# YonghaoHe/LFD-A-Light-and-Fast-Detector

Hardware: AMD Instinct MI355X
Metric: images/sec WIDERFACE-S 1920x1080 bs=8 end-to-end inference, LFD.precision='fp32_storage' (raw logits within 1e-4 of fp32: inside north_star's 1e-3; the 'fp16' mode, sigma 2.5e-3, under fp16_mode) (higher is better)
Workload: dtype f16

## Files before the change

### include/lfd_hip.h

```cpp
#ifndef LFD_HIP_H_
#define LFD_HIP_H_

#include <stddef.h>
#include <stdint.h>

#ifdef __cplusplus
extern "C" {
#endif

#define LFD_HIP_ABI_VERSION 3
#define LFD_MAX_LEVELS 8

typedef void* lfd_stream_t;

#if defined(LFD_BUILDING)
#define LFD_API __attribute__((visibility("default")))
#else
#define LFD_API
#endif

enum lfd_status {
  LFD_OK = 0,
  LFD_ERR_INVALID_ARGUMENT = -1,
  LFD_ERR_WORKSPACE_TOO_SMALL = -2,
// ... 201 lines not shown
                                    const float* b2, const void* zeros, lfd_stream_t stream);

LFD_API int lfd_upsample_nearest_add_nhwc_f16(void* dst, const void* src, int32_t n, int32_t H, int32_t W, int32_t h,
                                              int32_t w, int32_t c, lfd_stream_t stream);
LFD_API int lfd_relu_inplace_f16(void* x, int64_t count, lfd_stream_t stream);
LFD_API int lfd_maxpool3x3s2_nhwc_f16(const void* in, void* out, int32_t n, int32_t h, int32_t w, int32_t c,
                                      lfd_stream_t stream);
LFD_API int lfd_pack_level_outputs_f32(const float* src, float* dst, int32_t n, int32_t hw, int32_t src_channels, int32_t c0,
                                       int32_t count, int32_t total_points, int32_t point_offset, float scale, int32_t op,
                                       lfd_stream_t stream);

LFD_API int lfd_conv2d_nhwc_f16_acc32(const lfd_conv_desc_t* desc, const void* in, float* out_f32, const void* w_packed,
                                      const float* bias, const void* zeros, lfd_stream_t stream);

typedef struct lfd_p32_conv_desc {
  int32_t n, h, w, cin, cout, ks, stride, relu;
  int32_t in_format;
  int32_t out_pixel_stride;
  int64_t out_image_stride;
} lfd_p32_conv_desc_t;
LFD_API size_t lfd_p32_conv_packed_weight_halfs(int32_t cin, int32_t cout, int32_t ks);
LFD_API int lfd_p32_conv2d_nhwc_f32(const lfd_p32_conv_desc_t* desc, const void* in, float* out, const void* w_packed,
                                    const float* bias, const float* residual, const float* scale, lfd_stream_t stream);
LFD_API int lfd_p32_conv2d_tail_nhwc_f32(const lfd_p32_conv_desc_t* desc, const void* in, float* out, const void* w_packed,
                                         const float* bias, const void* tail_w_packed, const float* tail_bias, int32_t tail_relu,
                                         lfd_stream_t stream);
LFD_API size_t lfd_p32_groupnorm_workspace_bytes(int32_t n, int32_t groups);
LFD_API int lfd_p32_groupnorm_relu_f32(float* x, int32_t n, int64_t hw, int32_t c, int32_t groups, const float* gamma,
                                       const float* beta, float eps, int32_t relu, void* workspace, size_t workspace_bytes,
                                       lfd_stream_t stream);

#define LFD_PL_GN_REPLICAS 8
typedef struct lfd_pl_conv_desc {
  int32_t n, h, w, cin, cout, ks, stride, relu;
  int32_t tail_cout, tail_relu;
  int32_t out_mode;
  int32_t f_c0, f_c1;
  float gn_in_eps;
  int64_t in_plane_halfs, out_plane_halfs, res_plane_halfs, ds_plane_halfs;
  int64_t f_image_stride0, f_image_stride1;
} lfd_pl_conv_desc_t;
LFD_API int lfd_pl_stem_pair(const void* in, int32_t in_format, int32_t n, int32_t h, int32_t w, int32_t channels,
                             const void* w1_packed, const float* b1, const void* w2_packed, const float* b2, void* out,
                             int64_t out_plane_halfs, lfd_stream_t stream);
LFD_API int lfd_pl_stem2x(const void* in, int32_t in_format, int32_t n, int32_t h, int32_t w, const void* w1_packed,
                          const void* w2_packed, const float* b2, const void* w3_packed, const float* b3,
                          const void* w4_packed, const float* b4, void* out, int64_t out_plane_halfs, const void* zeros,
                          lfd_stream_t stream);
LFD_API int lfd_pl_conv2d(const lfd_pl_conv_desc_t* desc, const void* in, void* out, const void* w_packed, const float* bias,
                          const void* residual, const void* tail_w_packed, const float* tail_bias, const void* ds_w_packed,
                          const float* ds_bias, void* ds_out, void* gn_sums, float* f_out0, float* f_out1, const float* scale1,
                          const void* gn_in_sums, const float* gn_in_gamma, const float* gn_in_beta, const void* zeros,
                          lfd_stream_t stream);
typedef struct lfd_pl_level {
  const void* in;
  void* out;
  const void* w_packed;
  const float* bias;
  const void* tail_w_packed;
  const float* tail_bias;
  void* gn_sums;
  const void* gn_in_sums;
  const float* gn_in_gamma;
  const float* gn_in_beta;
  float* f_out0;
  float* f_out1;
  const float* scale1;
  int32_t h, w;
  int64_t in_plane_halfs, out_plane_halfs;
} lfd_pl_level_t;
LFD_API int lfd_pl_conv2d_levels(const lfd_pl_conv_desc_t* desc, const lfd_pl_level_t* levels, int32_t num_levels,
                                 const void* zeros, lfd_stream_t stream);
LFD_API int lfd_pl_groupnorm_relu(void* x, int64_t plane_halfs, int32_t n, int64_t hw, int32_t c, const void* gn_sums,
                                  const float* gamma, const float* beta, float eps, int32_t relu, lfd_stream_t stream);

typedef struct lfd_pl_head_desc {
  int32_t mode, n, cin, relu0;
  int32_t f_c0, f_c1;
  float gn_in_eps;
  int32_t pad_;
  int64_t f_image_stride0, f_image_stride1;
} lfd_pl_head_desc_t;
typedef struct lfd_pl_head_level {
  const void* in;
  void* out;
  const void* w0;
  const float* b0;
  const void* w1;
  const float* b1;
  void* gn_sums;
  const void* gn_in_sums;
  const float* gn_in_gamma;
  const float* gn_in_beta;
  float* f_out0;
  float* f_out1;
  const float* scale1;
  int64_t in_plane_halfs;
  int32_t pixels, pad_;
} lfd_pl_head_level_t;
LFD_API int lfd_pl_head_levels(const lfd_pl_head_desc_t* desc, const lfd_pl_head_level_t* levels, int32_t num_levels,
                               const void* zeros, lfd_stream_t stream);

LFD_API int lfd_stem_conv_f16(const void* in, int32_t in_format, int32_t n, int32_t h, int32_t w,
                              int32_t channels, const void* w1_packed, const float* b1,
                              const void* w2_packed, const float* b2, void* out, lfd_stream_t stream);

// ... 232 lines not shown
```

### lfd-a-light-and-fast-detector_amd/lfd_amd/_lib.py

```python
import ctypes as C
import os

_HERE = os.path.dirname(os.path.abspath(__file__))
LIB_PATH = os.environ.get('LFD_HIP_LIB') or os.path.join(_HERE, 'liblfd_hip.so')
MAX_LEVELS = 8
F32, F16 = 0, 1

_lib = None


class DetectDesc(C.Structure):
    _fields_ = [('num_levels', C.c_int32),
                ('level_h', C.c_int32 * MAX_LEVELS), ('level_w', C.c_int32 * MAX_LEVELS),
                ('level_stride', C.c_int32 * MAX_LEVELS),
                ('level_range_lo', C.c_float * MAX_LEVELS), ('level_range_hi', C.c_float * MAX_LEVELS),
                ('num_classes', C.c_int32), ('num_cls_channels', C.c_int32),
                ('score_mode', C.c_int32), ('decode_mode', C.c_int32),
                ('class_agnostic', C.c_int32), ('max_candidates', C.c_int32),
                ('score_thr', C.c_float), ('iou_thr', C.c_float)]


class DetectExt(C.Structure):
    _fields_ = [('pre_nms_limit', C.c_int32), ('post_nms_limit', C.c_int32)]

# ... 174 lines not shown
    'lfd_gn_train_stats_f16': (C.c_int, [_P, _I32, _I64, _I32, _I32, _F, _P, _SZ, _P, _P]),
    'lfd_gn_train_apply_f16': (C.c_int, [_P, _I32, _I64, _I32, _I32, _P, _P, _P, _I32, _P, _P]),
    'lfd_gn_train_stats_apply_f16': (C.c_int, [_P, _I32, _I64, _I32, _I32, _F, _P, _P, _I32, _P, _SZ, _P, _P, _P]),
    'lfd_gn_train_stats_apply_seg_f16': (C.c_int, [_P, _I32, _I32, _P, _I32, _I32, _F, _P, _P, _I32, _P, _SZ, _P, _P, _P]),
    'lfd_gn_train_bwd_seg_f16': (C.c_int, [_P, _P, _P, _I32, _I32, _P, _I32, _I32, _P, _P, _F, _I32, _P, _SZ, _P, _P, _P, _P]),
    'lfd_bn_train_apply_into_f16': (C.c_int, [_P, _I32, _I64, _I32, _P, _P, _P, _I32, _P, _I64, _I64, _P]),
    'lfd_bn_train_bwd_from_f16': (C.c_int, [_P, _I64, _I64, _P, _I32, _I32, _I64, _I32, _P, _P, _P, _F, _I32, _P, _SZ, _P, _P, _P, _P]),
    'lfd_head_out_split_concat_f16': (C.c_int, [_P, _I32, _I32, _I64, _I64, C.POINTER(HeadOutSeg), _I32, _P]),
    'lfd_head_out_grad_concat_f16': (C.c_int, [_P, _I32, _I32, _I64, _I64, C.POINTER(HeadOutSeg), _I32, _F, _P, _P, _SZ, _P]),
    'lfd_conv2d_bn_partials_nhwc_f16': (C.c_int, [C.POINTER(ConvDesc), _P, _P, _P, _P, _P, _P, _SZ, C.POINTER(C.c_int32), _P]),
    'lfd_bn_train_finish_into_levels_f16': (C.c_int, [C.POINTER(BnFwdLevel), _I32, _I32, _I32, _P, _I64, _P]),
    'lfd_bn_train_bwd_from_levels_f16': (C.c_int, [_P, _I64, C.POINTER(BnBwdLevel), _I32, _I32, _I32, _F, _I32, _P, _SZ, _P]),
    'lfd_head_out_split_levels_f16': (C.c_int, [_P, _I32, _I64, C.POINTER(HeadOutLevel), _I32, _P]),
    'lfd_head_out_grad_levels_f16': (C.c_int, [_P, _I32, _I64, C.POINTER(HeadOutLevel), _I32, _F, _P, _P, _SZ, _P]),
    'lfd_gn_train_bwd_f16': (C.c_int, [_P, _P, _P, _I32, _I64, _I32, _I32, _P, _P, _F, _I32, _P, _SZ, _P, _P, _P, _P]),
    'lfd_zero_insert2_nhwc_f16': (C.c_int, [_P, _I32, _I32, _I32, _I32, _I32, _I32, _P, _P]),
    'lfd_conv3x3s2_dgrad_nhwc_f16': (C.c_int, [_I32, _I32, _I32, _P, _P, _P, _P, _P]),
    'lfd_conv_wgrad_nhwc_f16': (C.c_int, [_P, _P, _I32, _I32, _I32, _I32, _I32, _I32, _I32, _F, _I32, _P, _SZ, _P, _P]),
    'lfd_conv_wgrad_partial_rows': (_I32, [_I32, _I32, _I32, _I32, _I32, _I32, _I32]),
    'lfd_conv_wgrad_partials_nhwc_f16': (C.c_int, [_P, _P, _I32, _I32, _I32, _I32, _I32, _I32, _I32, _P, _SZ, _P]),
    'lfd_conv1x1_wgrad_partials_of_bn_relu_f16': (C.c_int, [_P, _P, _P, _P, _P, _I32, _I32, _I32, _I32, _I32, _P, _SZ, _P]),
    'lfd_wgrad_final_batched_f32': (C.c_int, [_P, _I32, _I32, _P]),
    'lfd_rows_sum_batched_f32': (C.c_int, [_P, _I32, _P]),
    'lfd_stem_conv0_train_fwd': (C.c_int, [_P, _I32, _I32, _I32, _I32, _P, _P, _P]),
    'lfd_head_out_split_f16': (C.c_int, [_P, _I32, _I32, _I64, _I64, C.POINTER(HeadOutSeg), _I32, _P]),
    'lfd_head_out_grad_f16': (C.c_int, [_P, _I32, _I32, _I64, _I64, C.POINTER(HeadOutSeg), _I32, _F, _P, _P, _SZ, _P]),
    'lfd_stem_conv0_train_fwd_bn_stats': (C.c_int, [_P, _I32, _I32, _I32, _I32, _P, _P, _F, _F, _P, _P, _P, _SZ, _P, _P]),
    'lfd_stem_conv0_wgrad': (C.c_int, [_P, _P, _I32, _I32, _I32, _I32, _F, _I32, _P, _SZ, _P, _P]),
    'lfd_stem_conv0_bn_bwd_wgrad': (C.c_int, [_P, _P, _P, _I32, _I32, _I32, _I32, _P, _P, _P, _F, _I32, _P, _SZ, _P, _P, _P, _P]),
    'lfd_stem_conv0_bn_bwd_wgrad_rows': (C.c_int, [_P, _P, _P, _I32, _I32, _I32, _I32, _P, _P, _P, _F, _I32, _I32, _P, _SZ, _P, _P, _P, _P]),
    'lfd_bn_train_bwd_rows_f16': (C.c_int, [_P, _P, _I64, _I32, _P, _P, _P, _F, _I32, _I32, _P, _SZ, _P, _P, _P, _P]),
    'lfd_conv1x1_dgrad_bn_bwd_sums_nhwc_f16': (C.c_int, [C.POINTER(ConvDesc), _P, _P, _P, _P, _P, _P, _P, _P, _P, _P, _SZ, C.POINTER(C.c_int32), _P]),
    'lfd_stem_conv_f16': (C.c_int, [_P, _I32, _I32, _I32, _I32, _I32, _P, _P, _P, _P, _P, _P]),
    'lfd_stem_faster_fused_f16': (C.c_int, [_P, _I32, _I32, _I32, _I32, _I32, _P, _P, _P, _P, _P, _P, _P, _P, _P, _P]),
    'lfd_head_partial_floats': (_SZ, [C.POINTER(HeadDesc)]),
    'lfd_head_forward_f16': (C.c_int, [C.POINTER(HeadDesc), _I32, C.POINTER(HeadLevelPtrs), _P, _P, _P, _P, _P, _P, _P]),
    'lfd_head_forward_decode_f16': (C.c_int, [C.POINTER(HeadDesc), C.POINTER(HeadLevelPtrs), _P, _P, _P, _P, _P,
                                              C.POINTER(DetectDesc), _P, _P, _SZ, _P]),
    'lfd_groupnorm_finalize': (C.c_int, [C.POINTER(HeadDesc), _P, C.POINTER(C.c_void_p), C.POINTER(C.c_void_p), _F, _P, _P]),
    'lfd_groupnorm_finalize_fold': (C.c_int, [C.POINTER(HeadDesc), _P, C.POINTER(C.c_void_p), C.POINTER(C.c_void_p), _F, _P,
                                              C.POINTER(HeadLevelPtrs), _I32, _P]),
    'lfd_conv_packed_weight_halfs': (_SZ, [_I32, _I32, _I32]),
    'lfd_conv2d_nhwc_f16': (C.c_int, [C.POINTER(ConvDesc), _P, _P, _P, _P, _P, _P, _P, _P, _P]),
    'lfd_fasterblock_fused_f16': (C.c_int, [_I32, _I32, _I32, _P, _P, _P, _P, _P, _P, _P, _P]),
    'lfd_fasterblock128_fused_f16': (C.c_int, [_I32, _I32, _I32, _P, _P, _P, _P, _P, _P, _P]),
    'lfd_downblock_fused_f16': (C.c_int, [_I32, _I32, _I32, _P, _P, _P, _P, _P, _P, _P, _P, _P, _P]),
    'lfd_conv2d_nhwc_f16_acc32': (C.c_int, [C.POINTER(ConvDesc), _P, _P, _P, _P, _P, _P]),
    'lfd_p32_conv_packed_weight_halfs': (_SZ, [_I32, _I32, _I32]),
    'lfd_p32_conv2d_nhwc_f32': (C.c_int, [C.POINTER(P32ConvDesc), _P, _P, _P, _P, _P, _P, _P]),
    'lfd_p32_conv2d_tail_nhwc_f32': (C.c_int, [C.POINTER(P32ConvDesc), _P, _P, _P, _P, _P, _P, _I32, _P]),
    'lfd_pl_stem_pair': (C.c_int, [_P, _I32, _I32, _I32, _I32, _I32, _P, _P, _P, _P, _P, _I64, _P]),
    'lfd_pl_stem2x': (C.c_int, [_P, _I32, _I32, _I32, _I32, _P, _P, _P, _P, _P, _P, _P, _P, _I64, _P, _P]),
    'lfd_pl_conv2d': (C.c_int, [C.POINTER(PlConvDesc), _P, _P, _P, _P, _P, _P, _P, _P, _P, _P, _P, _P, _P, _P, _P, _P, _P, _P, _P]),
    'lfd_pl_conv2d_levels': (C.c_int, [C.POINTER(PlConvDesc), C.POINTER(PlLevel), _I32, _P, _P]),
    'lfd_pl_head_levels': (C.c_int, [C.POINTER(PlHeadDesc), C.POINTER(PlHeadLevel), _I32, _P, _P]),
    'lfd_pl_groupnorm_relu': (C.c_int, [_P, _I64, _I32, _I64, _I32, _P, _P, _P, _F, _I32, _P]),
    'lfd_p32_groupnorm_workspace_bytes': (_SZ, [_I32, _I32]),
    'lfd_p32_groupnorm_relu_f32': (C.c_int, [_P, _I32, _I64, _I32, _I32, _P, _P, _F, _I32, _P, _SZ, _P]),
    'lfd_conv2d_downsample_nhwc_f16': (C.c_int, [C.POINTER(ConvDesc), _P, _P, _P, _P, _P, _P, _P, _P, _P]),
}


TUNE_KEYS = {'HEAD2': 0, 'H2_CHUNK': 1, 'H2_AGPR': 2, 'H2_A1': 3, 'STEM2X': 4, 'X2_ALN': 5, 'X2_STAGGER': 6, 'BLOCK_ROWS': 7,
             'ROWS_WGS': 8, 'CONV128_SPLITK': 9, 'CONV0_VALU': 10, 'PL_C3': 11, 'PL_HEAD_OUT_REGS': 12, 'PL_HEAD_ROLES': 13, 'PL_STEM': 14}


def tune(name, value=None):
    key = TUNE_KEYS[name]
    prev = lib().lfd_tuning_get(key)
    if value is not None:
        check(lib().lfd_tuning_set(key, int(value)), 'lfd_tuning_set')
    return prev


def declared_symbols():
    return sorted(_SIGNATURES)


def lib():
    global _lib
    if _lib is None:
        if not os.path.exists(LIB_PATH):
            raise RuntimeError(
                'liblfd_hip.so not found at %s -- build it with `python __graft_entry__.py` '
                '(hipcc --offload-arch=gfx950); lfd_amd has no CPU/PyTorch fallback.' % LIB_PATH)
        import torch
        l = C.CDLL(LIB_PATH)
        for name, (res, args) in _SIGNATURES.items():
            fn = getattr(l, name)
            fn.restype, fn.argtypes = res, args
        if l.lfd_hip_abi_version() != ABI_VERSION:
            raise RuntimeError('liblfd_hip.so ABI version mismatch: %s reports %d, this package binds version %d '
                               '(struct layouts differ -- rebuild with `python __graft_entry__.py`)'
                               % (LIB_PATH, l.lfd_hip_abi_version(), ABI_VERSION))
        for name, key in TUNE_KEYS.items():
            v = os.environ.get('LFD_' + name)
            if v is not None and v.strip().lstrip('-').isdigit():
                l.lfd_tuning_set(key, int(v))
        _lib = l
    return _lib


def check(status, what):
    if status != 0:
        raise RuntimeError('%s failed: %s (status %d)' % (what, lib().lfd_hip_status_string(status).decode(), status))

# ... 15 lines not shown
```

### lfd-a-light-and-fast-detector_amd/lfd_amd/engine_p2.py

```python
import ctypes as C
import os

import torch
import torch.nn as nn

from . import _lib, engine, ops
from ._lib import check, lib, ptr, stream_ptr

_UNION = engine._UNION
_LO = 2048.0


class Unsupported(Exception):
    pass


def _split(w):
    w = w.detach().float()
    hi = w.half()
    lo = ((w - hi.float()) * _LO).half()
    return hi, lo


def pack_planes_weight(w):
# ... 1 lines not shown
    cout = w.shape[0]
    ns = -(-cout // 32)
    if ns * 32 != cout:
        w = torch.cat([w, w.new_zeros((ns * 32 - cout,) + tuple(w.shape[1:]))], 0)
    hi, lo = _split(w)
    return torch.stack([ops.pack_conv_weight(hi), ops.pack_conv_weight(lo)], 0).contiguous()


def pack_planes_stem_weight(w):
    hi, lo = _split(w)
    return torch.stack([engine.pack_stem_weight(hi), engine.pack_stem_weight(lo)], 0).contiguous()


def pack_planes_stem2x_weight(w, b):
    if tuple(w.shape) != (64, 3, 3, 3) or b.numel() != 64:
        raise Unsupported('fused stem: conv0 must be [64, 3, 3, 3]')
    c = 64
    wr = w.detach().float().permute(0, 2, 3, 1).reshape(c // 32, 32, 3, 9)
    out = torch.zeros(c // 32, 2, 2, 32, 8, dtype=torch.float32, device=w.device)
    out[:, 0, 0, :, 1:] = wr[:, :, 0, :7]
    out[:, 0, 1, :, 1:] = wr[:, :, 2, :7]
    out[:, 1, 0, :, 1:] = wr[:, :, 1, :7]
    for r in range(3):
        out[:, 1, 1, :, 2 * r:2 * r + 2] = wr[:, :, r, 7:9]
    out[:, 1, 1, :, 6] = b.detach().float().reshape(c // 32, 32).to(w.device)
    hi, lo = _split(out.reshape(c // 32, 2, 64, 8))
    return torch.stack([hi, lo], 0).contiguous()


def pack_planes_stem2x_tail_weight(w):
    if tuple(w.shape) != (64, 64, 1, 1):
        raise Unsupported('fused stem: first 1x1 must be [64, 64, 1, 1]')
    w2 = w.detach().float().reshape(64, 64)
    idx = torch.empty(4, 2, 8, dtype=torch.long)
    for q in range(4):
        s_, u = q // 2, q % 2
        for hh in range(2):
            for j in range(8):
                idx[q, hh, j] = 32 * s_ + 16 * u + (4 * hh + j if j < 4 else 8 + 4 * hh + j - 4)
    g = w2[:, idx.reshape(-1).to(w2.device)].reshape(2, 32, 4, 2, 8)
    out = g.permute(0, 2, 3, 1, 4).reshape(2, 4, 64, 8)
    hi, lo = _split(out)
    return torch.stack([hi, lo], 0).contiguous()


def _flat_head_enabled():
    return os.environ.get('LFD_P2_FLATHEAD', '1') != '0'


def _stem2x_enabled():
    return os.environ.get('LFD_P2_STEM2X', '1') != '0'


def _pad_bias(b, mult=32):
    n = -(-b.numel() // mult) * mult
    out = b.new_zeros(n, dtype=torch.float32)
    out[:b.numel()] = b.float()
    return out


def to_planes(x):
    hi = x.half()
    return torch.stack([hi, ((x - hi.float()) * _LO).half()], 0).contiguous()


def from_planes(p):
    return p[0].float() + p[1].float() / _LO


_DISPATCH = {
    (64, 3, 1, 2): {'res'}, (64, 3, 2, 2): {'tail', 'ds'}, (64, 3, 2, 4): {'ds'}, (64, 1, 1, 4): {'tail', 'gn', 'out32'},
    (128, 3, 1, 4): {'res'}, (128, 3, 2, 4): {'ds'}, (128, 1, 1, 4): {'tail', 'gn', 'out32'}, (128, 1, 1, 1): {'out32'},
    (128, 1, 1, 2): {'out32'}, (32, 3, 2, 1): {'tail', 'ds'}, (32, 3, 2, 2): {'tail', 'ds'},
}


def _check_dispatch(cin, cout, ks, stride, tail, ds, res, gn, out32):
    opts = _DISPATCH.get((cin, ks, stride, -(-cout // 32)))
    used = {k for k, v in (('tail', tail), ('ds', ds), ('res', res), ('gn', gn), ('out32', out32)) if v}
    if opts is None or not (used - {'gn'} <= opts and (not gn or 'gn' in opts)) or len(used - {'gn'}) > 1:
        raise Unsupported('no plane kernel for conv %d -> %d k%d s%d %s' % (cin, cout, ks, stride, sorted(used)))
    if gn and (res or ds or out32):
        raise Unsupported('GroupNorm sums ride on a plain or chained 1x1')


def _fork_enabled():
    import os
    return os.environ.get('LFD_P2_FORK', '0') != '0'


def _levels_enabled():
    return os.environ.get('LFD_P2_LEVELS', '1') != '0'


class _Op(object):
    __slots__ = ('kind', 'src', 'dst', 'res', 'ds_dst', 'cin', 'cout', 'ks', 'stride', 'relu', 'w', 'b', 'tail', 'ds',
                 'out_mode', 'gn', 'gnin', 'level', 'f_c0', 'f_c1', 'scale', 'w1', 'b1', 'w2', 'b2', 'channels')

    def __init__(self, kind):
        self.kind = kind
        for k in self.__slots__[1:]:
            setattr(self, k, None)


class PlanesPlan(object):

    def __init__(self, model, device):
        self.device = device
        self.param_sig = engine._param_signature(model._backbone, model._neck, model._head)
        self._shape_cache = {}
        self.ops = []
        self.buf_channels = {}
        self.buf_scale = {}
        self._nbuf = 0
        self.num_gn = 0
        self.head_start = None
        self.level_ops = []
        self.tap_ready = []
        with torch.no_grad():
            self._build(model)

    def _new_buf(self, channels, scale):
        b = self._nbuf
        self._nbuf += 1
        self.buf_channels[b], self.buf_scale[b] = channels, scale
        return b

    def _conv(self, src, w, b, ks, stride, relu, res=None, tail=None, ds=None, gn=False, out32=None, gnin=None):
        dev = self.device
        cout, cin = w.shape[0], w.shape[1]
        if cin not in (32, 64, 128) or (out32 is None and cout % 32):
            raise Unsupported('conv %d -> %d' % (cin, cout))
        _check_dispatch(cin, cout, ks, stride, tail is not None, ds is not None, res is not None, gn, out32 is not None)
        o = _Op('conv')
        if gnin is not None:
            norm = gnin[1]
            if not (isinstance(norm, nn.GroupNorm) and norm.num_channels == 128 and norm.num_groups == 16 and cin == 128 and ks == 1
                    and stride == 1 and tail is None and res is None and ds is None):
                raise Unsupported('head norm must be GroupNorm(16, 128) in front of a 1x1 conv')
            o.gnin = (gnin[0], norm.weight.detach().float().contiguous().to(dev), norm.bias.detach().float().contiguous().to(dev),
                      float(norm.eps))
        o.src, o.res, o.ks, o.stride, o.relu, o.cin, o.cout = src, res, ks, stride, int(relu), cin, cout
        o.w = pack_planes_weight(w).to(dev)
        o.b = _pad_bias(b, 128).to(dev)
        sc = self.buf_scale[src] * stride
        if tail is not None:
            if tuple(tail[0].shape) != (cout, cout, 1, 1):
                raise Unsupported('chained 1x1 must be square')
            o.tail = (pack_planes_weight(tail[0]).to(dev), _pad_bias(tail[1], 128).to(dev), int(tail[2]))
        if ds is not None:
            if tuple(ds[0].shape) != (cout, cin, 1, 1) or ks != 3 or stride != 2:
                raise Unsupported('identity branch must be the 1x1 stride-2 twin of a 3x3 stride-2 conv')
            o.ds = (pack_planes_weight(ds[0]).to(dev), _pad_bias(ds[1], 128).to(dev))
            o.ds_dst = self._new_buf(cout, sc)
        if out32 is not None:
            o.out_mode = 2
            o.level, o.f_c0, o.f_c1, o.scale = out32
        else:
            o.out_mode = 1 if gn else 0
            o.dst = self._new_buf(cout, sc)
            if gn:
                if cout != 128:
                    raise Unsupported('GroupNorm sums: 128 channels in groups of 8')
                o.gn = self.num_gn
                self.num_gn += 1
        self.ops.append(o)
        return o

    def _build(self, model):
        bb, neck, head = model._backbone, model._neck, model._head
        if type(neck).__name__ != 'SimpleNeck' or type(head).__name__ != 'LFDHead':
# ... 6 lines not shown
                        'Conv2d', 'BatchNorm2d', 'GroupNorm', 'ReLU', 'Scale', 'Identity', 'Sequential', 'ModuleList'):
                    raise Unsupported('module %s (activation must be ReLU)' % type(mod).__name__)
        has_norm = bb._norm_cfg is not None
        step = 3 if has_norm else 2
        spec = list(bb.stem_spec())
        folded = [engine.fold_conv_norm(bb._stem[i * step], bb._stem[i * step + 1] if has_norm else None) for i in range(len(spec))]
        if len(spec) not in (2, 4) or [(k, s) for k, s, _, _ in spec] != [(3, 2), (1, 1)] * (len(spec) // 2):
            raise Unsupported('stem mode')
        c = folded[0][0].shape[0]
        if c not in (32, 64) or tuple(folded[1][0].shape[:2]) != (c, c):
            raise Unsupported('stem channels')
        o = _Op('stem')
        o.channels = c
        o.w1, o.b1 = pack_planes_stem_weight(folded[0][0]).to(self.device), _pad_bias(folded[0][1]).to(self.device)
        o.w2, o.b2 = pack_planes_weight(folded[1][0]).to(self.device), _pad_bias(folded[1][1]).to(self.device)
        o.dst = self._new_buf(c, 2)
        self.ops.append(o)
        cur = o.dst
        self.stem2x = None
        if len(spec) == 4:
            if tuple(folded[3][0].shape[:2]) != (c, c):
                raise Unsupported('stem channels')
            pair2 = self._conv(cur, folded[2][0], folded[2][1], 3, 2, True, tail=(folded[3][0], folded[3][1], True))
            cur = pair2.dst
            if c == 64:
                f = _Op('stem2x')
                f.w1 = pack_planes_stem2x_weight(folded[0][0], folded[0][1]).to(self.device)
                f.w2, f.b2 = pack_planes_stem2x_tail_weight(folded[1][0]).to(self.device), o.b2
                f.dst = cur
                f.tail = pair2
                self.stem2x = f
        taps = [tuple(t) for t in bb._out_indices]
        self.taps = []
        for i, nblk in enumerate(bb._body_architecture):
            for j in range(nblk):
                blk = getattr(bb, 'stage%d' % i)[j]
                ident, y = cur, cur
                for ci in range(1, blk.num_convs + 1):
                    conv = getattr(blk, '_conv%d' % ci)
                    w, b = engine.fold_conv_norm(conv, getattr(blk, '_norm%d' % ci, None))
                    ks, st = conv.kernel_size[0], conv.stride[0]
                    last = ci == blk.num_convs
                    ds = None
                    if ci == 1 and blk._downsample is not None:
                        dconv = blk._downsample[0]
                        if dconv.kernel_size[0] != 1 or dconv.stride[0] != 2 or (ks, st) != (3, 2) or last:
                            raise Unsupported('downsample branch')
                        ds = engine.fold_conv_norm(dconv, blk._downsample[1] if len(blk._downsample) > 1 else None)
                    elif ci > 1 and st != 1:
                        raise Unsupported('stride inside a block')
                    if ci == 1 and blk._downsample is None and st != 1:
                        raise Unsupported('strided block without a downsample branch')
                    op = self._conv(y, w, b, ks, st, True, res=ident if last else None, ds=ds)
                    y = op.dst
                    if ds is not None:
                        ident = op.ds_dst
                cur = y
                if (i, j) in taps:
                    self.taps.append(cur)
                    self.tap_ready.append(len(self.ops) - 1)
        if head._norm_cfg is None or head._conv_kernel_size != 1:
            raise Unsupported('head towers must be 1x1 conv + GroupNorm')
        nl = head._num_conv_layers
        union = head._regression_loss_type in _UNION
        self.cls_channels = head.num_cls_channels
        self.num_levels = head._num_heads
        ccls = self.cls_channels

        def tower(seq, t, first_tail_of=None):
            pend = None
            for l in range(nl):
                conv, norm = seq[l * 3], seq[l * 3 + 1]
                if not isinstance(norm, nn.GroupNorm):
                    raise Unsupported('head norm must be GroupNorm')
                if not isinstance(seq[l * 3 + 2], nn.ReLU):
                    raise Unsupported('head activation must be ReLU')
                bias = conv.bias.detach().float() if conv.bias is not None else torch.zeros(conv.out_channels, device=conv.weight.device)
                w = conv.weight.detach().float()
                if l == 0 and first_tail_of is not None:
                    nw, nb, src = first_tail_of
                    op = self._conv(src, nw, nb, 1, 1, True, tail=(w, bias, False), gn=True)
                else:
                    op = self._conv(t, w, bias, 1, 1, False, gn=True, gnin=pend)
                pend = (op.gn, norm)
                t = op.dst
            return t, pend

        self.head_start = len(self.ops)
        for i, f in enumerate(self.taps):
            first_op = len(self.ops)
            nseq = getattr(neck, 'neck%d' % i)
            nw, nb = engine.fold_conv_norm(nseq[0], nseq[1] if neck._norm_cfg is not None else None)
            if nw.shape[0] != 128 or nw.shape[2] != 1:
                raise Unsupported('neck must be 1x1 -> 128')
            cls_path = getattr(head, 'head%d_classification_path' % i)
            reg_path = getattr(head, 'head%d_regression_path' % i)
            scale = head._scales[i]._scale.detach().float().reshape(1).to(self.device) if union else None
            if head._merge_path_flag:
                if nl < 1:
                    raise Unsupported('merge path without tower convs')
                tt, pend = tower(getattr(head, 'head%d_merge_path' % i), None, first_tail_of=(nw, nb, f))
                cconv, rconv = cls_path[0], reg_path[0]
                if cconv.kernel_size[0] != 1 or rconv.kernel_size[0] != 1 or ccls + 4 > 64:
                    raise Unsupported('output convs')
                w = torch.cat([cconv.weight.detach().float(), rconv.weight.detach().float()], 0)
                b = torch.cat([cconv.bias.detach().float(), rconv.bias.detach().float()], 0)
# ... 157 lines not shown
                    d.mode, d.n, d.cin, d.relu0 = mode, st.n, o.cin, o.relu
                    if mode == 0:
                        lv.w1, lv.b1 = o.tail[0].data_ptr(), o.tail[1].data_ptr()
                    if mode != 2:
                        lv.out, lv.gn_sums = st.bufs[o.dst].data_ptr(), st.gn_sums[o.gn].data_ptr()
                    if gi is not None:
                        lv.gn_in_sums, lv.gn_in_gamma, lv.gn_in_beta = st.gn_sums[gi[0]].data_ptr(), gi[1].data_ptr(), gi[2].data_ptr()
                        d.gn_in_eps = gi[3]
                    if mode == 2:
                        d.f_c0, d.f_c1 = o.f_c0, o.f_c1
                        d.f_image_stride0, d.f_image_stride1 = st.P * o.f_c0, st.P * 4
                        lv.f_out0 = (st.cls.data_ptr() + st.p_off[o.level] * o.f_c0 * 4) if o.f_c0 else None
                        lv.f_out1 = (st.reg.data_ptr() + st.p_off[o.level] * 4 * 4) if o.f_c1 else None
                        lv.scale1 = o.scale.data_ptr() if o.scale is not None else None
                calls.append((mode, d, arr, len(grp)))
            st.flat_calls = calls
        for mode, d, arr, n in st.flat_calls:
            if mode == 'G':
                check(l.lfd_pl_conv2d_levels(C.byref(d), arr, n, zeros, sp), 'lfd_pl_conv2d_levels')
            else:
                check(l.lfd_pl_head_levels(C.byref(d), arr, n, zeros, sp), 'lfd_pl_head_levels')

    def _launch_levels(self, st):
        modes = self._flat_head_modes() if _flat_head_enabled() else None
        if modes is not None:
            return self._launch_levels_flat(st, modes)
        l, sp = lib(), stream_ptr()
        zeros = ptr(ops.zero_line(self.device))
        if st.level_calls is None:
            calls = []
            for grp in self.level_groups:
                arr = (_lib.PlLevel * len(grp))()
                d0 = None
                for j, i in enumerate(grp):
                    o = self.ops[i]
                    d, src, dst, _, _, f0, f1 = self._desc(o, st)
                    d0 = d0 or d
                    lv, gi = arr[j], o.gnin
                    lv.in_, lv.out, lv.w_packed, lv.bias = src.data_ptr(), dst.data_ptr() if dst is not None else None, o.w.data_ptr(), o.b.data_ptr()
                    if o.tail is not None:
                        lv.tail_w_packed, lv.tail_bias = o.tail[0].data_ptr(), o.tail[1].data_ptr()
                    if o.gn is not None:
                        lv.gn_sums = st.gn_sums[o.gn].data_ptr()
                    if gi is not None:
                        lv.gn_in_sums, lv.gn_in_gamma, lv.gn_in_beta = st.gn_sums[gi[0]].data_ptr(), gi[1].data_ptr(), gi[2].data_ptr()
                    lv.f_out0, lv.f_out1 = f0, f1
                    lv.scale1 = o.scale.data_ptr() if o.scale is not None else None
                    lv.h, lv.w, lv.in_plane_halfs, lv.out_plane_halfs = src.shape[2], src.shape[3], d.in_plane_halfs, d.out_plane_halfs
                calls.append((d0, arr, len(grp)))
            st.level_calls = calls
        for d, arr, n in st.level_calls:
            check(l.lfd_pl_conv2d_levels(C.byref(d), arr, n, zeros, sp), 'lfd_pl_conv2d_levels')

    def _launch(self, x, fmt, st, indices):
        l, sp = lib(), stream_ptr()
        zeros = ptr(ops.zero_line(self.device))
        fused = (self.stem2x is not None and _stem2x_enabled() and
                 (os.environ.get('LFD_P2_STEM2X') == '2' or
                  (x.data_ptr() % 16 == 0 and ((fmt == 1 and st.w % 8 == 0) or (fmt == 2 and st.w % 16 == 0) or (fmt == 0 and st.w % 4 == 0)))))
        for i in indices:
            o = self.ops[i]
            if fused and i < 2:
                if i == 0:
                    f, c2 = self.stem2x, self.stem2x.tail
                    dst = st.bufs[f.dst]
                    check(l.lfd_pl_stem2x(ptr(x), fmt, st.n, st.h, st.w, ptr(f.w1), ptr(f.w2), ptr(f.b2), ptr(c2.w), ptr(c2.b),
                                          ptr(c2.tail[0]), ptr(c2.tail[1]), ptr(dst), dst[0].numel(), zeros, sp), 'lfd_pl_stem2x')
                continue
            if o.kind == 'stem':
                dst = st.bufs[o.dst]
                check(l.lfd_pl_stem_pair(ptr(x), fmt, st.n, st.h, st.w, o.channels, ptr(o.w1), ptr(o.b1), ptr(o.w2), ptr(o.b2),
                                         ptr(dst), dst[0].numel(), sp), 'lfd_pl_stem_pair')
                continue
            d, src, dst, res, dsd, f0, f1 = self._desc(o, st)
            gi = o.gnin
            check(l.lfd_pl_conv2d(C.byref(d), ptr(src), ptr(dst), ptr(o.w), ptr(o.b), ptr(res),
                                  ptr(o.tail[0]) if o.tail else None, ptr(o.tail[1]) if o.tail else None,
                                  ptr(o.ds[0]) if o.ds else None, ptr(o.ds[1]) if o.ds else None, ptr(dsd),
                                  ptr(st.gn_sums[o.gn]) if o.gn is not None else None, f0, f1,
                                  ptr(o.scale) if o.scale is not None else None,
                                  ptr(st.gn_sums[gi[0]]) if gi else None, ptr(gi[1]) if gi else None, ptr(gi[2]) if gi else None,
                                  zeros, sp), 'lfd_pl_conv2d')


class _LazyBufs(dict):

    def __init__(self, st, plan):
        super().__init__()
        self._st, self._plan = st, plan

    def __missing__(self, b):
        hh, ww = self._st.dims[b]
        with torch.cuda.device(self._plan.device):
            t = torch.empty((2, self._st.n, hh, ww, self._plan.buf_channels[b]), dtype=torch.float16, device=self._plan.device)
        self[b] = t
        return t


class _State(object):

    def __init__(self, plan, n, h, w):
        dev = plan.device
        self.n, self.h, self.w = n, h, w
        self.dims = {}
        self.bufs = _LazyBufs(self, plan)
        with torch.cuda.device(dev):
            for b, sc in plan.buf_scale.items():
                hh, ww, s = h, w, sc
                while s > 1:
                    hh, ww = (hh + 1) // 2, (ww + 1) // 2
                    s //= 2
                self.dims[b] = (hh, ww)
            self.sizes = [self.dims[t] for t in plan.taps]
            self.p_off, p = [], 0
# ... 12 lines not shown
```

Measured before the change: 6490.

## Fuse 64-channel residual block's two 3x3 convs into one pipelined kernel

Adds a fused HIP kernel that computes both 3x3 64-channel convolutions of a residual block in one launch. The intermediate activation stays in an LDS row ring, and the residual add is done with identity-matrix MFMAs. Waves are split into producer and consumer roles working a row pipeline. This removes the round trip of the intermediate tensor through global memory and one launch per block, in exchange for recomputing halo rows and running one workgroup per CU with heavy LDS use. It is enabled only when the PL_C3 tuning value equals 2.

```diff
diff --git a/include/lfd_hip.h b/include/lfd_hip.h
--- a/include/lfd_hip.h
+++ b/include/lfd_hip.h
@@ -277,6 +277,9 @@
                           const float* ds_bias, void* ds_out, void* gn_sums, float* f_out0, float* f_out1, const float* scale1,
                           const void* gn_in_sums, const float* gn_in_gamma, const float* gn_in_beta, const void* zeros,
                           lfd_stream_t stream);
+LFD_API int lfd_pl_block64(int32_t n, int32_t h, int32_t w, const void* in, int64_t in_plane_halfs, void* out,
+                           int64_t out_plane_halfs, const void* w1_packed, const float* b1, const void* w2_packed,
+                           const float* b2, const void* zeros, lfd_stream_t stream);
 typedef struct lfd_pl_level {
   const void* in;
   void* out;
diff --git a/lfd-a-light-and-fast-detector_amd/csrc/planes_block.hip b/lfd-a-light-and-fast-detector_amd/csrc/planes_block.hip
--- /dev/null
+++ b/lfd-a-light-and-fast-detector_amd/csrc/planes_block.hip
@@ -0,0 +1,302 @@
+#include "planes_impl.h"
+
+namespace pl {
+namespace {
+
+struct BlkArgs {
+  const _Float16* in;
+  long in_plane;
+  _Float16* out;
+  long out_plane;
+  const half8* w1;
+  const float* b1;
+  const half8* w2;
+  const float* b2;
+  const _Float16* zeros;
+  int N, H, W;
+  int strips, segs, SH, nwork;
+};
+
+struct PB {
+  static constexpr int TW = 30, IW = 34;
+  static constexpr int PIXB = 144;
+  static constexpr int NDMA = 5;
+  static constexpr int IN_PLANE = IW * PIXB + 256;
+  static constexpr int IN_SLOT = 2 * IN_PLANE;
+  static constexpr int NIN = 8;
+  static constexpr int MID_PLANE = IW * PIXB;
+  static constexpr int MID_SLOT = 2 * MID_PLANE;
+  static constexpr int NMID = 4;
+  static constexpr int NK = 36, KA = 18, KB = NK - KA;
+  static constexpr int LEAD = 5;
+  static constexpr int XCH = 64 * 16 * 4;
+  static constexpr int OFF_IN = 0;
+  static constexpr int OFF_MID = OFF_IN + NIN * IN_SLOT;
+  static constexpr int OFF_X1 = OFF_MID + NMID * MID_SLOT;
+  static constexpr int OFF_X2 = OFF_X1 + 4 * XCH;
+  static constexpr int OFF_BIAS = OFF_X2 + 4 * XCH;
+  static constexpr int LDS_BYTES = OFF_BIAS + 2 * 64 * 4;
+};
+static_assert(pl::PB::LDS_BYTES <= 160 * 1024, "LDS capacity");
+static_assert(pl::PB::NIN >= pl::PB::LEAD + 3 && pl::PB::NMID >= 4, "ring depths (see the header)");
+
+struct PSeg { int n, oy0, ox0, R; };
+
+__device__ __forceinline__ void pb_issue_row(const BlkArgs& a, char* smem, const PSeg& sg, int plane, int il, int slot) {
+  const int ol = threadIdx.x & 63;
+  const int px = (ol * 57) >> 9;
+  const int ck = ol - 9 * px;
+  const bool lane_on = ck < 8 && ol < 63;
+  const int gy = sg.oy0 - 2 + il;
+  const bool rv = gy >= 0 && gy < a.H && il < sg.R + 4;
+  const char* rowp = reinterpret_cast<const char*>(a.in + (size_t)plane * a.in_plane) +
+                     ((long)sg.n * a.H + (rv ? gy : 0)) * (long)a.W * 128;
+  const char* zp = reinterpret_cast<const char*>(a.zeros) + (ck & 7) * 16;
+  char* lrow = smem + pl::PB::OFF_IN + slot * pl::PB::IN_SLOT + plane * pl::PB::IN_PLANE;
+#pragma unroll
+  for (int i = 0; i < pl::PB::NDMA; ++i) {
+    const int col = 7 * i + px;
+    const int gx = sg.ox0 - 2 + col;
+    const bool ok = rv && gx >= 0 && gx < a.W;
+    const char* src = ok ? rowp + (long)gx * 128 + (ck & 7) * 16 : zp;
+    if (lane_on && col < pl::PB::IW) dma16(src, lrow + i * 1008);
+  }
+}
+
+__device__ __forceinline__ half8 pb_identity_fragment(int pix, int h, int qq) {
+  int j0 = pix - 16 * qq - 8 * h;
+  asm volatile("" : "+v"(j0));
+  union { half8 v; uint32_t u[4]; } f;
+#pragma unroll
+  for (int r = 0; r < 4; ++r) f.u[r] = (j0 == 2 * r) ? 0x3c00u : ((j0 == 2 * r + 1) ? 0x3c000000u : 0u);
+  return f.v;
+}
+
+template <bool CONV2, bool B>
+__device__ __forceinline__ void pb_role(const BlkArgs& a, char* smem, int ct, const PSeg& sg) {
+  const int lane = threadIdx.x & 63;
+  const int h = lane >> 5, pix = lane & 31;
+  constexpr int K0 = B ? pl::PB::KA : 0;
+  constexpr int KN = B ? pl::PB::KB : pl::PB::KA;
+  constexpr int PD = 2;
+  constexpr bool DMA = !CONV2 && !B;
+  const int T = sg.R + 5;
+  const int row_lag = CONV2 ? 4 : 0;
+  const int nrows = CONV2 ? sg.R : sg.R + 2;
+
+  if (DMA) {
+    for (int il = 0; il < pl::PB::LEAD; ++il) pb_issue_row(a, smem, sg, ct, il, il);
+  }
+  half8 wh[KN], wl[KN];
+  {
+    const half8* wsrc = (CONV2 ? a.w2 : a.w1) + (size_t)(ct * pl::PB::NK + K0) * 64 + lane;
+    constexpr long WPL = 2L * pl::PB::NK * 64;
+#pragma unroll
+    for (int k = 0; k < KN; ++k) {
+      wh[k] = wsrc[(size_t)k * 64];
+      wl[k] = wsrc[WPL + (size_t)k * 64];
+    }
+  }
+  const float* sbias = reinterpret_cast<const float*>(smem + pl::PB::OFF_BIAS) + (CONV2 ? 64 : 0);
+  float* xch = reinterpret_cast<float*>(smem + (CONV2 ? pl::PB::OFF_X2 : pl::PB::OFF_X1)) + ct * (pl::PB::XCH / 4) + lane * 4;
+  const int RING = CONV2 ? pl::PB::NMID : pl::PB::NIN;
+  const int SLOT = CONV2 ? pl::PB::MID_SLOT : pl::PB::IN_SLOT;
+  const int PLANE = CONV2 ? pl::PB::MID_PLANE : pl::PB::IN_PLANE;
+  const char* ring = smem + (CONV2 ? pl::PB::OFF_MID : pl::PB::OFF_IN) + pix * pl::PB::PIXB + h * 16;
+
+  float yp[16];
+#pragma unroll
+  for (int r = 0; r < 16; ++r) yp[r] = 0.f;
+
+  block_barrier();
+  for (int j = 0; j < T; ++j) {
+    if (DMA) asm volatile("s_waitcnt vmcnt(%0)" ::"n"(2 * pl::PB::NDMA) : "memory");
+    block_barrier();
+    const int r0 = j - row_lag;
+    if constexpr (B) {
+      const int re = r0 - 1;
+      if (re >= 0 && re < nrows) {
+        const float* xr = xch + ((j - 1) & 1) * (pl::PB::XCH / 2);
+        float y[16];
+#pragma unroll
+        for (int g = 0; g < 4; ++g) {
+          const float4 pa = *reinterpret_cast<const float4*>(xr + g * 256);
+          y[4 * g + 0] = fmaxf(yp[4 * g + 0] + pa.x, 0.f);
+          y[4 * g + 1] = fmaxf(yp[4 * g + 1] + pa.y, 0.f);
+          y[4 * g + 2] = fmaxf(yp[4 * g + 2] + pa.z, 0.f);
+          y[4 * g + 3] = fmaxf(yp[4 * g + 3] + pa.w, 0.f);
+        }
+        if constexpr (!CONV2) {
+          const int my = sg.oy0 - 1 + re, mx = sg.ox0 - 1 + pix;
+          const bool inimg = my >= 0 && my < a.H && mx >= 0 && mx < a.W;
+          char* mid = smem + pl::PB::OFF_MID + (re % pl::PB::NMID) * pl::PB::MID_SLOT + pix * pl::PB::PIXB + ct * 64 + h * 8;
+#pragma unroll
+          for (int g = 0; g < 4; ++g) {
+            uint2 vh, vl;
+            split2(y[4 * g + 0], y[4 * g + 1], vh.x, vl.x);
+            split2(y[4 * g + 2], y[4 * g + 3], vh.y, vl.y);
+            if (!inimg) { vh = uint2{0u, 0u}; vl = uint2{0u, 0u}; }
+            *reinterpret_cast<uint2*>(mid + 16 * g) = vh;
+            *reinterpret_cast<uint2*>(mid + pl::PB::MID_PLANE + 16 * g) = vl;
+          }
+        } else {
+          const int oy = sg.oy0 + re, ox = sg.ox0 + pix;
+          if (pix < pl::PB::TW && ox < a.W) {
+            _Float16* o = a.out + (((size_t)sg.n * a.H + oy) * a.W + ox) * 64 + ct * 32 + 4 * h;
+#pragma unroll
+            for (int g = 0; g < 4; ++g) {
+              uint2 vh, vl;
+              split2(y[4 * g + 0], y[4 * g + 1], vh.x, vl.x);
+              split2(y[4 * g + 2], y[4 * g + 3], vh.y, vl.y);
+              *reinterpret_cast<uint2*>(o + 8 * g) = vh;
+              *reinterpret_cast<uint2*>(o + a.out_plane + 8 * g) = vl;
+            }
+          }
+        }
+      }
+    }
+    if (r0 >= 0 && r0 < nrows) {
+      f32x16 am, ac;
+      if constexpr (!B) {
+        const float* bp = sbias + ct * 32 + 4 * h;
+#pragma unroll
+        for (int g = 0; g < 4; ++g) {
+          const float4 b4 = *reinterpret_cast<const float4*>(bp + 8 * g);
+          am[4 * g + 0] = b4.x; am[4 * g + 1] = b4.y; am[4 * g + 2] = b4.z; am[4 * g + 3] = b4.w;
+        }
+#pragma unroll
+        for (int r = 0; r < 16; ++r) ac[r] = 0.f;
+      } else {
+#pragma unroll
+        for (int r = 0; r < 16; ++r) am[r] = ac[r] = 0.f;
+      }
+      int rb[3];
+#pragma unroll
+      for (int r = 0; r < 3; ++r) rb[r] = ((r0 + r) % RING) * SLOT;
+      auto xaddr = [&](int k) {
+        const int r = k / 12, s = (k / 4) % 3, q = k % 4;
+        return ring + rb[r] + s * pl::PB::PIXB + q * 32;
+      };
+      half8 xqh[PD + 1], xql[PD + 1];
+#pragma unroll
+      for (int k = 0; k < PD; ++k) {
+        const char* p = xaddr(K0 + k);
+        xqh[k] = *reinterpret_cast<const half8*>(p);
+        xql[k] = *reinterpret_cast<const half8*>(p + PLANE);
+      }
+      static_for([&](auto kc) {
+        constexpr int k = decltype(kc)::value;
+        if constexpr (k + PD < KN) {
+          const char* p = xaddr(K0 + k + PD);
+          xqh[(k + PD) % (PD + 1)] = *reinterpret_cast<const half8*>(p);
+          xql[(k + PD) % (PD + 1)] = *reinterpret_cast<const half8*>(p + PLANE);
+        }
+        PL_SB();
+        am = __builtin_amdgcn_mfma_f32_32x32x16_f16(wh[k], xqh[k % (PD + 1)], am, 0, 0, 0);
+        ac = __builtin_amdgcn_mfma_f32_32x32x16_f16(wh[k], xql[k % (PD + 1)], ac, 0, 0, 0);
+        ac = __builtin_amdgcn_mfma_f32_32x32x16_f16(wl[k], xqh[k % (PD + 1)], ac, 0, 0, 0);
+        PL_SB();
+      }, std::make_integer_sequence<int, KN>{});
+      if constexpr (CONV2 && !B) {
+        const char* ib = smem + pl::PB::OFF_IN + ((r0 + 2) % pl::PB::NIN) * pl::PB::IN_SLOT + (pix + 2) * pl::PB::PIXB + ct * 64 + h * 16;
+#pragma unroll
+        for (int qq = 0; qq < 2; ++qq) {
+          const half8 rh = *reinterpret_cast<const half8*>(ib + qq * 32);
+          const half8 rl = *reinterpret_cast<const half8*>(ib + pl::PB::IN_PLANE + qq * 32);
+          const half8 idf = pb_identity_fragment(pix, h, qq);
+          am = __builtin_amdgcn_mfma_f32_32x32x16_f16(idf, rh, am, 0, 0, 0);
+          ac = __builtin_amdgcn_mfma_f32_32x32x16_f16(idf, rl, ac, 0, 0, 0);
+        }
+      }
+      if constexpr (!B) {
+        float* xw = xch + (j & 1) * (pl::PB::XCH / 2);
+#pragma unroll
+        for (int g = 0; g < 4; ++g) {
+          float4 v;
+          v.x = comb(am[4 * g + 0], ac[4 * g + 0]);
+          v.y = comb(am[4 * g + 1], ac[4 * g + 1]);
+          v.z = comb(am[4 * g + 2], ac[4 * g + 2]);
+          v.w = comb(am[4 * g + 3], ac[4 * g + 3]);
+          *reinterpret_cast<float4*>(xw + g * 256) = v;
+        }
+      } else {
+#pragma unroll
+        for (int r = 0; r < 16; ++r) yp[r] = comb(am[r], ac[r]);
+      }
+    }
+    if (DMA) pb_issue_row(a, smem, sg, ct, j + pl::PB::LEAD, (j + pl::PB::LEAD) % pl::PB::NIN);
+  }
+}
+
+__global__ __launch_bounds__(512, 1) void k_pl_blk64(BlkArgs a) {
+  extern __shared__ __attribute__((aligned(16))) char smem[];
+  const int wave = __builtin_amdgcn_readfirstlane((int)(threadIdx.x >> 6));
+  if (threadIdx.x < 128) {
+    float* sb = reinterpret_cast<float*>(smem + pl::PB::OFF_BIAS);
+    sb[threadIdx.x] = threadIdx.x < 64 ? a.b1[threadIdx.x] : a.b2[threadIdx.x - 64];
+  }
+  const int w = blockIdx.x;
+  PSeg sg;
+  {
+    const int per_img = a.segs * a.strips;
+    sg.n = w / per_img;
+    const int r = w - sg.n * per_img;
+    const int seg = r / a.strips, strip = r - seg * a.strips;
+    sg.oy0 = seg * a.SH;
+    sg.ox0 = strip * pl::PB::TW;
+    sg.R = (a.H - sg.oy0) < a.SH ? (a.H - sg.oy0) : a.SH;
+  }
+  switch (wave) {
+    case 0: case 1: pb_role<false, false>(a, smem, wave, sg); break;
+    case 2: case 3: pb_role<false, true>(a, smem, wave - 2, sg); break;
+    case 4: case 5: pb_role<true, true>(a, smem, wave - 4, sg); break;
+    default: pb_role<true, false>(a, smem, wave - 6, sg); break;
+  }
+}
+
+}
+}
+
+extern "C" LFD_API int lfd_pl_block64(int32_t n, int32_t h, int32_t w, const void* in, int64_t in_plane_halfs, void* out,
+                                      int64_t out_plane_halfs, const void* w1_packed, const float* b1, const void* w2_packed,
+                                      const float* b2, const void* zeros, lfd_stream_t stream) {
+  if (!in || !out || !w1_packed || !b1 || !w2_packed || !b2 || !zeros) return LFD_ERR_INVALID_ARGUMENT;
+  if (n < 1 || h < 1 || w < 1) return LFD_ERR_INVALID_ARGUMENT;
+  if (!lfd_aligned16(in) || !lfd_aligned16(out) || !lfd_aligned16(w1_packed) || !lfd_aligned16(w2_packed))
+    return LFD_ERR_INVALID_ARGUMENT;
+  if ((long)(h) * w * 64 * 2 > 0x7fffffffL) return LFD_ERR_UNSUPPORTED;
+  const long plane = (long)n * h * w * 64;
+  if (in_plane_halfs < plane || out_plane_halfs < plane || (in_plane_halfs & 7) || (out_plane_halfs & 7))
+    return LFD_ERR_INVALID_ARGUMENT;
+  const char *ib = (const char*)in, *ob = (const char*)out;
+  if (ib < ob + 2 * out_plane_halfs * 2 && ob < ib + 2 * in_plane_halfs * 2) return LFD_ERR_INVALID_ARGUMENT;
+  pl::BlkArgs a{};
+  a.in = (const _Float16*)in; a.in_plane = in_plane_halfs;
+  a.out = (_Float16*)out; a.out_plane = out_plane_halfs;
+  a.w1 = (const half8*)w1_packed; a.b1 = b1; a.w2 = (const half8*)w2_packed; a.b2 = b2;
+  a.zeros = (const _Float16*)zeros;
+  a.N = n; a.H = h; a.W = w;
+  static unsigned long long attr_done_mask = 0;
+  const int dev = lfd_device_ordinal();
+  if (LFD_ONCE_PER_DEVICE(attr_done_mask, dev)) {
+    if (hipFuncSetAttribute(reinterpret_cast<const void*>(&pl::k_pl_blk64), hipFuncAttributeMaxDynamicSharedMemorySize,
+                            pl::PB::LDS_BYTES) != hipSuccess)
+      return LFD_ERR_LAUNCH_FAILED;
+    LFD_DONE_ON_DEVICE(attr_done_mask, dev);
+  }
+  a.strips = (w + pl::PB::TW - 1) / pl::PB::TW;
+  const long cols = (long)n * a.strips;
+  int segs = (int)(256 / cols);
+  if (segs < 1) segs = 1;
+  int sh = (h + segs - 1) / segs;
+  if (sh < 4) sh = 4;
+  if (sh > h) sh = h;
+  a.SH = sh;
+  a.segs = (h + sh - 1) / sh;
+  const long nwork = cols * a.segs;
+  if (nwork > 0x7fffffffL) return LFD_ERR_UNSUPPORTED;
+  a.nwork = (int)nwork;
+  hipLaunchKernelGGL(pl::k_pl_blk64, dim3(a.nwork), dim3(512), pl::PB::LDS_BYTES, (hipStream_t)stream, a);
+  LFD_CHECK_LAUNCH();
+  return LFD_OK;
+}
diff --git a/lfd-a-light-and-fast-detector_amd/lfd_amd/_lib.py b/lfd-a-light-and-fast-detector_amd/lfd_amd/_lib.py
--- a/lfd-a-light-and-fast-detector_amd/lfd_amd/_lib.py
+++ b/lfd-a-light-and-fast-detector_amd/lfd_amd/_lib.py
@@ -250,6 +250,7 @@
     'lfd_pl_stem_pair': (C.c_int, [_P, _I32, _I32, _I32, _I32, _I32, _P, _P, _P, _P, _P, _I64, _P]),
     'lfd_pl_stem2x': (C.c_int, [_P, _I32, _I32, _I32, _I32, _P, _P, _P, _P, _P, _P, _P, _P, _I64, _P, _P]),
     'lfd_pl_conv2d': (C.c_int, [C.POINTER(PlConvDesc), _P, _P, _P, _P, _P, _P, _P, _P, _P, _P, _P, _P, _P, _P, _P, _P, _P, _P, _P]),
+    'lfd_pl_block64': (C.c_int, [_I32, _I32, _I32, _P, _I64, _P, _I64, _P, _P, _P, _P, _P, _P]),
     'lfd_pl_conv2d_levels': (C.c_int, [C.POINTER(PlConvDesc), C.POINTER(PlLevel), _I32, _P, _P]),
     'lfd_pl_head_levels': (C.c_int, [C.POINTER(PlHeadDesc), C.POINTER(PlHeadLevel), _I32, _P, _P]),
     'lfd_pl_groupnorm_relu': (C.c_int, [_P, _I64, _I32, _I64, _I32, _P, _P, _P, _F, _I32, _P]),
diff --git a/lfd-a-light-and-fast-detector_amd/lfd_amd/engine_p2.py b/lfd-a-light-and-fast-detector_amd/lfd_amd/engine_p2.py
--- a/lfd-a-light-and-fast-detector_amd/lfd_amd/engine_p2.py
+++ b/lfd-a-light-and-fast-detector_amd/lfd_amd/engine_p2.py
@@ -77,6 +77,10 @@
     return os.environ.get('LFD_P2_STEM2X', '1') != '0'
 
 
+def _block_enabled():
+    return os.environ.get('LFD_P2_BLOCK', '1') != '0'
+
+
 def _pad_bias(b, mult=32):
     n = -(-b.numel() // mult) * mult
     out = b.new_zeros(n, dtype=torch.float32)
@@ -142,6 +146,7 @@
         self.head_start = None
         self.level_ops = []
         self.tap_ready = []
+        self.block_pairs = {}
         with torch.no_grad():
             self._build(model)
 
@@ -254,6 +259,11 @@
                     if ci == 1 and blk._downsample is None and st != 1:
                         raise Unsupported('strided block without a downsample branch')
                     op = self._conv(y, w, b, ks, st, True, res=ident if last else None, ds=ds)
+                    if (ci == 2 and last and blk._downsample is None and self.ops[-2].dst == y and self.ops[-2].src == ident and
+                            op.res == ident and
+                            all(q.ks == 3 and q.stride == 1 and q.cin == 64 and q.cout == 64 and q.relu and q.tail is None
+                                and q.ds is None and q.out_mode == 0 for q in self.ops[-2:])):
+                        self.block_pairs[len(self.ops) - 2] = len(self.ops) - 1
                     y = op.dst
                     if ds is not None:
                         ident = op.ds_dst
@@ -517,14 +527,29 @@
         for d, arr, n in st.level_calls:
             check(l.lfd_pl_conv2d_levels(C.byref(d), arr, n, zeros, sp), 'lfd_pl_conv2d_levels')
 
+    def _fused_block(self, st):
+        return bool(self.block_pairs) and _block_enabled() and _lib.tune('PL_C3') == 2
+
     def _launch(self, x, fmt, st, indices):
         l, sp = lib(), stream_ptr()
         zeros = ptr(ops.zero_line(self.device))
+        fblk = self._fused_block(st)
+        blk_second = set(self.block_pairs.values()) if fblk else ()
         fused = (self.stem2x is not None and _stem2x_enabled() and
                  (os.environ.get('LFD_P2_STEM2X') == '2' or
                   (x.data_ptr() % 16 == 0 and ((fmt == 1 and st.w % 8 == 0) or (fmt == 2 and st.w % 16 == 0) or (fmt == 0 and st.w % 4 == 0)))))
         for i in indices:
             o = self.ops[i]
+            if fblk:
+                if i in blk_second:
+                    continue
+                j = self.block_pairs.get(i)
+                if j is not None:
+                    o2 = self.ops[j]
+                    src, dst = st.bufs[o.src], st.bufs[o2.dst]
+                    check(l.lfd_pl_block64(st.n, src.shape[2], src.shape[3], ptr(src), src[0].numel(), ptr(dst), dst[0].numel(),
+                                           ptr(o.w), ptr(o.b), ptr(o2.w), ptr(o2.b), zeros, sp), 'lfd_pl_block64')
+                    continue
             if fused and i < 2:
                 if i == 0:
                     f, c2 = self.stem2x, self.stem2x.tail
```

Result: faster. 6822 (median of 6 runs) (+5.1%).
